# ChuRuaNh0/Image_Restoration

Hardware: AMD Instinct MI355X
Metric: images/sec (128x128->512x512 x4 SR, 23-block RRDBNet) (higher is better)
Workload: dtype f32

## Files before the change

### image_restoration_amd/csrc/conv_wino_f32.hip

```cpp
#include <stdlib.h>

#include <type_traits>

#include "sr_internal.h"

typedef float f32x4 __attribute__((ext_vector_type(4)));
typedef float f32x16 __attribute__((ext_vector_type(16)));

namespace {

struct WinoParams {
  const float* in;
  const float* u;
  const float* bias;
  float* out;
  const float* res1;
  const float* res2;
  long long in_ns, out_ns, res1_ns, res2_ns;
  int cin_blocks, cout_blocks;
  int in_h, in_w;
  int H, W;
  int tiles_x, tiles_y;
  int src_shift;
  int res_cb1;
  float slope, alpha, beta1, beta2;
#ifdef SR_WINO_STAMP
  unsigned long long* stamps;
#endif
};

#ifdef SR_WINO_STAMP
#define WINO_STAMP(k)                                                                                               \
  do {                                                                                                              \
    if (p.stamps && wave == 0 && lane == 0)                                                                         \
      p.stamps[(size_t)(blockIdx.y * gridDim.x + blockIdx.x) * 8 + (k)] = __builtin_amdgcn_s_memtime();             \
  } while (0)
#else
#define WINO_STAMP(k) \
  do {                \
  } while (0)
#endif

constexpr int XROW = 66;

template <int NW>
constexpr int wino_x_bytes() {
  return (((2 * NW + 2) * XROW * 32 + NW * 1024 - 1) / (NW * 1024)) * (NW * 1024);
}
template <int NW>
constexpr int wino_lds_bytes() {
  return 3 * wino_x_bytes<NW>() + 2 * 16 * 1024;
}

template <int NW, int HF>
__device__ __forceinline__ void conv_wino_tile_f32(const WinoParams p, char* smem, const int wave) {
  constexpr int NV = 2 * NW;
  constexpr int XPIX = (2 * NW + 2) * XROW;
  constexpr int XBYTES = wino_x_bytes<NW>();
  constexpr int NXU = (XPIX * 32 + 1023) / 1024, NWU = 16;
  constexpr int NXR = (NXU + NV - 1) / NV, NWR = NWU / NV;
  static_assert(NV * 8192 <= 3 * XBYTES, "the exchange of the output transform lives in the X buffers");

  int t;
  {
    const int nwg = gridDim.x, b = blockIdx.x;
    const int xcd = b & 7, q = nwg >> 3, r = nwg & 7;
    t = (xcd < r ? xcd * (q + 1) : r * (q + 1) + (xcd - r) * q) + (b >> 3);
  }
  const int tx = t % p.tiles_x;
  t /= p.tiles_x;
  const int ty = t % p.tiles_y;
  const int n = t / p.tiles_y;
  const int cog = blockIdx.y;

  const int lane = threadIdx.x & 63;
  WINO_STAMP(0);
  const int prow = wave - HF * NW;
  const int j = lane & 31, h = lane >> 5;
  const int x0 = tx * 64, y0 = ty * (2 * NW);
  const int HWin = p.in_h * p.in_w;
  const float* in_n = p.in + (long long)n * p.in_ns;
  const float* ug = p.u + (size_t)cog * p.cin_blocks * (NWU * 256);

  unsigned xvo[NXR];
#pragma unroll
  for (int r = 0; r < NXR; ++r) {
    const int u = r * NV + wave;
    const int q = u * 64 + lane;
    const int pix = q >> 1, half = q & 1;
    const int row = pix / XROW, col = pix - row * XROW;
    const int gy = y0 - 1 + row, gx = x0 - 1 + col;
    const bool valid = pix < XPIX && gy >= 0 && gy < p.H && gx >= 0 && gx < p.W;
    const int sy = gy >> p.src_shift, sx = gx >> p.src_shift;
    const int hsw = half ^ ((col >> 3) & 1);
    xvo[r] = valid ? (unsigned)((sy * p.in_w + sx) * 8 + hsw * 4) * 4u : 0xfffffff0u;
  }
  const __amdgpu_buffer_rsrc_t x_rs =
      __builtin_amdgcn_make_buffer_rsrc((void*)in_n, 0, (unsigned)((long long)p.cin_blocks * HWin * 32), 0x00020000);
  const __amdgpu_buffer_rsrc_t u_rs =
      __builtin_amdgcn_make_buffer_rsrc((void*)ug, 0, (unsigned)((long long)p.cin_blocks * NWU * 1024), 0x00020000);
  const unsigned uvo = (lane ^ ((lane >> 4) & 1)) * 16;
  auto stage_x = [&](int buf, int cb) {
    char* xs = smem + buf * XBYTES;
    const unsigned xso = (unsigned)cb * (unsigned)HWin * 32u;
#pragma unroll
    for (int r = 0; r < NXR; ++r) {
      const int u = r * NV + wave;
      if ((r + 1) * NV <= NXU || u < NXU)
        __builtin_amdgcn_raw_ptr_buffer_load_lds(x_rs, (__attribute__((address_space(3))) void*)(xs + u * 1024), 16, xvo[r], xso, 0, 0);
    }
  };
  auto stage_u = [&](int buf, int cb) {
    char* us = smem + 3 * XBYTES + buf * (NWU * 1024);
    const unsigned uso = (unsigned)cb * (NWU * 1024u);
#pragma unroll
    for (int r = 0; r < NWR; ++r) {
      const int u = r * NV + wave;
      __builtin_amdgcn_raw_ptr_buffer_load_lds(u_rs, (__attribute__((address_space(3))) void*)(us + u * 1024), 16, uvo, uso + u * 1024u, 0, 0);
    }
  };

  f32x16 acc[8];
#pragma unroll
  for (int a = 0; a < 8; ++a)
#pragma unroll
    for (int e = 0; e < 16; ++e) acc[a][e] = 0.f;

  int xlane[4];
#pragma unroll
  for (int c = 0; c < 4; ++c) xlane[c] = ((2 * prow + HF) * XROW + 2 * j + c) * 32 + ((h ^ (((2 * j + c) >> 3) & 1)) * 16);
  const int ulane = HF * 8 * 1024 + j * 32 + ((h ^ ((j >> 3) & 1)) * 16);

  f32x4 tr[2][4], v[8];
  auto rows = [&](int buf) {
    const char* xb = smem + buf * XBYTES;
#pragma unroll
    for (int c = 0; c < 4; ++c) {
      const f32x4 e0 = *(const f32x4*)(xb + xlane[c]);
      const f32x4 e1 = *(const f32x4*)(xb + xlane[c] + XROW * 32);
      const f32x4 e2 = *(const f32x4*)(xb + xlane[c] + 2 * XROW * 32);
      if constexpr (HF == 0) {
        tr[0][c] = e0 - e2;
        tr[1][c] = e1 + e2;
      } else {
        tr[0][c] = e1 - e0;
        tr[1][c] = e0 - e2;
      }
    }
  };
  auto cols = [&](int r) {
    v[r * 4 + 0] = tr[r][0] - tr[r][2];
    v[r * 4 + 1] = tr[r][1] + tr[r][2];
    v[r * 4 + 2] = tr[r][2] - tr[r][1];
    v[r * 4 + 3] = tr[r][1] - tr[r][3];
  };

  const int nchunk = p.cin_blocks;
  stage_x(0, 0);
  stage_u(0, 0);
  if (nchunk > 1) stage_x(1, 1);
  __syncthreads();
  WINO_STAMP(1);
  rows(0);
#pragma unroll
  for (int r = 0; r < 2; ++r) cols(r);
  int xb2 = 2 % 3, xb1 = 1;
  auto chunk = [&](int c, auto more_t, auto more2_t) {
    constexpr bool more = decltype(more_t)::value, more2 = decltype(more2_t)::value;
    const char* us = smem + 3 * XBYTES + (c & 1) * (NWU * 1024) + ulane;
    f32x4 a[2][4];
#pragma unroll
    for (int q = 0; q < 4; ++q) a[0][q] = *(const f32x4*)(us + q * 1024);
#pragma unroll
    for (int g = 0; g < 2; ++g) {
      if (g == 0) {
#pragma unroll
        for (int q = 0; q < 4; ++q) a[1][q] = *(const f32x4*)(us + (4 + q) * 1024);
        if constexpr (more2) stage_x(xb2, c + 2);
        if constexpr (more) stage_u((c + 1) & 1, c + 1);
      }
#pragma unroll
      for (int s = 0; s < 4; ++s)
#pragma unroll
        for (int q = 0; q < 4; ++q)
          acc[g * 4 + q] = __builtin_amdgcn_mfma_f32_32x32x2f32(a[g][q][s], v[g * 4 + q][s], acc[g * 4 + q], 0, 0, 0);
      if constexpr (more) {
        if (g == 0) rows(xb1);
        else cols(0);
      }
      __builtin_amdgcn_sched_barrier(0);
    }
    if constexpr (more) cols(1);
    __syncthreads();
    xb1 = xb2;
    xb2 = xb2 == 2 ? 0 : xb2 + 1;
  };
  using yes = std::true_type;
  using no = std::false_type;
  for (int c = 0; c + 2 < nchunk; ++c) chunk(c, yes{}, yes{});
  if (nchunk > 1) chunk(nchunk - 2, yes{}, no{});
  chunk(nchunk - 1, no{}, no{});
  WINO_STAMP(2);

  f32x16 ra[2][2];
#pragma unroll
  for (int r = 0; r < 2; ++r) {
    ra[r][0] = (acc[r * 4 + 0] + acc[r * 4 + 1]) + acc[r * 4 + 2];
    ra[r][1] = (acc[r * 4 + 1] - acc[r * 4 + 2]) - acc[r * 4 + 3];
  }

  f32x16 yv[2];
  {
    char* mine = smem + wave * 8192 + lane * 16;
    const char* theirs = smem + (HF ? wave - NW : wave + NW) * 8192 + lane * 16;
#pragma unroll
    for (int c = 0; c < 2; ++c)
#pragma unroll
      for (int k = 0; k < 4; ++k) {
        f32x4 o;
#pragma unroll
        for (int e = 0; e < 4; ++e) o[e] = ra[1 - HF][c][k * 4 + e];
        *(f32x4*)(mine + (c * 4 + k) * 1024) = o;
      }
    __syncthreads();
#pragma unroll
    for (int c = 0; c < 2; ++c) {
      f32x16 rb;
#pragma unroll
      for (int k = 0; k < 4; ++k) {
        const f32x4 o = *(const f32x4*)(theirs + (c * 4 + k) * 1024);
#pragma unroll
        for (int e = 0; e < 4; ++e) rb[k * 4 + e] = o[e];
      }
      if constexpr (HF == 0) yv[c] = (ra[0][c] + ra[1][c]) + rb;
      else yv[c] = (rb - ra[0][c]) - ra[1][c];
    }
  }

  WINO_STAMP(3);

  const long long HW = (long long)p.H * p.W;
  const int y = y0 + 2 * prow + HF;
#pragma unroll
  for (int dx = 0; dx < 2; ++dx) {
    const int x = x0 + 2 * j + dx;
    if (y >= p.H || x >= p.W) continue;
    const long long pixoff = (long long)y * p.W + x;
#pragma unroll
    for (int g = 0; g < 4; ++g) {
      const int cb = cog * 4 + g;
      if (cb >= p.cout_blocks) continue;
      f32x4 o;
#pragma unroll
      for (int e = 0; e < 4; ++e) o[e] = yv[dx][g * 4 + e];
      const long long off = (cb * HW + pixoff) * 8 + h * 4;
      if (p.bias) o += *(const f32x4*)(p.bias + cb * 8 + h * 4);
#pragma unroll
      for (int e = 0; e < 4; ++e) o[e] = o[e] > 0.f ? o[e] : o[e] * p.slope;
      o *= p.alpha;
      if (p.res1 && cb < p.res_cb1) o += p.beta1 * *(const f32x4*)(p.res1 + (long long)n * p.res1_ns + off);
      if (p.res2 && cb < p.res_cb1) o += p.beta2 * *(const f32x4*)(p.res2 + (long long)n * p.res2_ns + off);
      *(f32x4*)(p.out + (long long)n * p.out_ns + off) = o;
    }
  }
  WINO_STAMP(4);
}

template <int NW>
__global__ __launch_bounds__(NW * 128, 2) void conv_wino_f32_kernel(const WinoParams p) {
  extern __shared__ __attribute__((aligned(16))) char smem[];
  const int wave = __builtin_amdgcn_readfirstlane(threadIdx.x >> 6);
  if (wave < NW) conv_wino_tile_f32<NW, 0>(p, smem, wave);
  else conv_wino_tile_f32<NW, 1>(p, smem, wave);
}

#ifdef SR_WINO_STAMP
unsigned long long* g_wino_stamps = nullptr;
#endif

template <int NW>
int launch_wino(const WinoParams& p0, const sr_conv3x3_desc* d, hipStream_t stream) {
  WinoParams p = p0;
#ifdef SR_WINO_STAMP
  p.stamps = g_wino_stamps;
#endif
  p.tiles_x = sr::cdiv(p.W, 64);
  p.tiles_y = sr::cdiv(p.H, 2 * NW);
  constexpr int lds = wino_lds_bytes<NW>();
  auto kern = conv_wino_f32_kernel<NW>;
  if (int rc = sr::ensure_dynamic_lds((const void*)kern, lds)) return rc;
  const int groups = d->cout / 32;
  const bool prof = sr::prof_on();
  if (prof) {
    sr_launch_record r = {};
    r.kernel_id = NW == 4 ? 106 : NW == 2 ? 107 : 108;
    r.cin = d->cin_real > 0 ? d->cin_real : d->cin_pad;
    r.cout = d->cout;
    r.n = d->n;
    r.h = p.H;
    r.w = p.W;
    const double px = (double)d->n * p.H * p.W;
    const double patches = (double)d->n * ((p.H + 1) / 2) * ((p.W + 1) / 2);
    r.flops = 2.0 * 16 * d->cin_pad * d->cout * patches;
    double fl = (double)d->n * p.in_h * p.in_w * r.cin + px * r.cout;
    if (d->res1) fl += px * r.cout;
    if (d->res2) fl += px * r.cout;
    r.bytes = 4.0 * fl;
    sr::prof_begin(stream, r);
  }
  hipLaunchKernelGGL(kern, dim3(p.tiles_x * p.tiles_y * d->n, groups), dim3(NW * 128), lds, stream, p);
  if (prof) sr::prof_end(stream);
  SR_CHECK_LAUNCH("conv_wino_f32 launch");
  return SR_OK;
}

int g_wino_mode = -1;

}

namespace sr {

int wino_f32_mode() {
  if (g_wino_mode < 0) {
    const char* e = getenv("SR_F32_WINOGRAD");
    g_wino_mode = (e && *e) ? atoi(e) : 1;
    if (g_wino_mode < 0 || g_wino_mode > 4) g_wino_mode = 1;
  }
  return g_wino_mode;
}

bool wino_f32_weights_eligible(int cout, int cin) { return cin >= 8 && cout > 0 && cout % 32 == 0; }

size_t wino_f32_image_floats(int cout, int cin_pad) { return (size_t)cout * cin_pad * 16; }

int conv3x3_wino_f32(const sr_conv3x3_desc* d, const float* image, hipStream_t stream, bool any_size) {
  SR_CHECK_ARG(d != nullptr && image != nullptr, "conv3x3_wino_f32: null argument");
  SR_CHECK_ARG(d->in && d->out, "conv3x3_wino_f32: null in/out");
  SR_CHECK_ARG(d->cin_pad > 0 && d->cin_pad % 8 == 0, "conv3x3_wino_f32: cin_pad=%d must be a positive multiple of 8", d->cin_pad);
  SR_CHECK_ARG(d->cout > 0 && d->n > 0 && d->in_h > 0 && d->in_w > 0, "conv3x3_wino_f32: bad shape");
  SR_CHECK_ARG(((uintptr_t)d->in | (uintptr_t)image | (uintptr_t)d->out | (uintptr_t)d->res1 | (uintptr_t)d->res2 | (uintptr_t)d->bpacked) % 16 == 0,
               "conv3x3_wino_f32: pointers must be 16-byte aligned");
  const int cin = d->cin_real > 0 ? d->cin_real : d->cin_pad;
  if (!wino_f32_weights_eligible(d->cout, cin) || d->out_nchw || d->accumulate || d->mask_src || d->s2_channels || d->out_unshuffle2 ||
      d->res1_u2 || d->res1_keep_sign || (d->upsample != 0 && d->upsample != 1))
    return SR_WINO_NOT_ELIGIBLE;
  WinoParams p = {};
  p.in = d->in;
  p.u = image;
  p.bias = d->bpacked;
  p.out = d->out;
  p.res1 = d->res1;
  p.res2 = d->res2;
  p.in_ns = d->in_img_stride;
  p.out_ns = d->out_img_stride;
  p.res1_ns = d->res1_img_stride;
  p.res2_ns = d->res2_img_stride;
  p.cin_blocks = d->cin_pad / 8;
  p.cout_blocks = d->cout / 8;
  p.in_h = d->in_h;
  p.in_w = d->in_w;
  p.src_shift = d->upsample ? 1 : 0;
  p.H = d->in_h << p.src_shift;
  p.W = d->in_w << p.src_shift;
  p.res_cb1 = d->res_cbn > 0 ? d->res_cbn : (1 << 30);
  p.slope = d->act_slope;
  p.alpha = d->alpha;
  p.beta1 = d->beta1;
  p.beta2 = d->beta2;
  const long long blocks = p.cout_blocks > p.cin_blocks ? p.cout_blocks : p.cin_blocks;
  if ((long long)p.H * p.W * 32 * blocks >= (1ll << 31) || (long long)p.in_h * p.in_w * 32 * blocks >= (1ll << 31))
    return SR_WINO_NOT_ELIGIBLE;
  const int mode = wino_f32_mode();
  if (!any_size && mode < 2 && (long long)p.H * p.W < 128 * 128) return SR_WINO_NOT_ELIGIBLE;
  const long long rows2 = cdiv(p.H, 4), rows1 = cdiv(p.H, 2);
  const long long per_row = (long long)cdiv(p.W, 64) * d->n * (d->cout / 32) * launch_concurrency();
  if (per_row * rows1 >= (1ll << 31)) return SR_WINO_NOT_ELIGIBLE;
  const int nw = mode >= 2 ? (mode == 2 ? 4 : mode == 3 ? 2 : 1) : rows2 * per_row >= 256 ? 2 : 1;
  return nw == 4 ? launch_wino<4>(p, d, stream) : nw == 2 ? launch_wino<2>(p, d, stream) : launch_wino<1>(p, d, stream);
}

}

extern "C" int sr_dev_set_wino_f32(int mode) {
  g_wino_mode = (mode >= 0 && mode <= 4) ? mode : 1;
  return SR_OK;
}

#ifdef SR_WINO_STAMP
extern "C" int sr_dev_set_wino_stamps(unsigned long long* buf) {
  g_wino_stamps = buf;
  return SR_OK;
}
#endif

extern "C" int sr_dev_conv3x3_wino_f32(const sr_conv3x3_desc* d, const float* wino_image, void* stream) {
  return sr::conv3x3_wino_f32(d, wino_image, (hipStream_t)stream, true);
}

extern "C" size_t sr_dev_conv3x3_wino_packed_floats(int cout, int cin_pad) {
  return (cout > 0 && cin_pad > 0 && cout % 32 == 0 && cin_pad % 8 == 0) ? sr::wino_f32_image_floats(cout, cin_pad) : 0;
}

extern "C" int sr_dev_conv3x3_wino_pack_f32(const float* weight, int cout, int cin, int first_seg, int seg, float* wino_image,
                                            void* stream) {
  SR_CHECK_ARG(weight && wino_image && sr::wino_f32_weights_eligible(cout, cin), "sr_dev_conv3x3_wino_pack_f32: bad argument");
  const int cin_pad = sr_conv3x3_cin_pad(cin, first_seg, seg);
  SR_CHECK_ARG(cin_pad > 0, "sr_dev_conv3x3_wino_pack_f32: cin=%d is not first_seg=%d + k*seg=%d", cin, first_seg, seg);
  std::vector<sr::PackEntry> tab(1);
  sr::PackEntry& e = tab[0];
  e = sr::PackEntry{};
  e.kind = 3;
  e.w[0] = weight;
  e.out = wino_image;
  e.cout = cout;
  e.cin = cin;
  e.first_seg = first_seg;
  e.seg = seg > 0 ? seg : 1;
  e.cin_pad = cin_pad;
  return sr::pack_table_run(tab, wino_image, sr::wino_f32_image_floats(cout, e.cin_pad) * sizeof(float), false, (hipStream_t)stream);
}

extern "C" size_t sr_dev_conv3x3_wino_pack_bytes(int cout, int cin_pad) {
  const size_t f = sr_dev_conv3x3_wino_packed_floats(cout, cin_pad);
  return f ? f * sizeof(float) + sr::pack_table_bytes(1) : 0;
}
```

Baseline: 411.8.

## Add nearest-upsample Winograd variant skipping zero tiles and stage residual via LDS

Adds a specialised Winograd F(2x2,3x3) kernel for the nearest-neighbour x2 upsample conv (src_shift==1). It exploits duplicated input rows and columns so that 7 of the 16 transformed elements are zero, and skips their loads, transforms, MFMAs and the cross-half exchange. For NW<=2 it also prefetches the res1 residual tile into the X region of LDS during the last chunk, and moves the output-transform exchange into the U buffers. The cost is more template instantiations and LDS reuse constraints, and the UP2 algebra must be correct.

```diff
diff --git a/image_restoration_amd/csrc/conv_wino_f32.hip b/image_restoration_amd/csrc/conv_wino_f32.hip
--- a/image_restoration_amd/csrc/conv_wino_f32.hip
+++ b/image_restoration_amd/csrc/conv_wino_f32.hip
@@ -52,14 +52,19 @@
   return 3 * wino_x_bytes<NW>() + 2 * 16 * 1024;
 }
 
-template <int NW, int HF>
+template <int NW, int HF, bool UP2>
 __device__ __forceinline__ void conv_wino_tile_f32(const WinoParams p, char* smem, const int wave) {
   constexpr int NV = 2 * NW;
   constexpr int XPIX = (2 * NW + 2) * XROW;
   constexpr int XBYTES = wino_x_bytes<NW>();
   constexpr int NXU = (XPIX * 32 + 1023) / 1024, NWU = 16;
   constexpr int NXR = (NXU + NV - 1) / NV, NWR = NWU / NV;
-  static_assert(NV * 8192 <= 3 * XBYTES, "the exchange of the output transform lives in the X buffers");
+  constexpr bool RES_LDS = NW <= 2;
+  constexpr int RBYTES = NV * 8 * 1024;
+  constexpr int XCH = RES_LDS ? 3 * XBYTES : 0;
+  auto used = [](int a) constexpr { return !UP2 || ((a & 3) != 2 && !(HF == 1 && (a >> 2) == 0)); };
+  static_assert(RES_LDS ? (NV * 8192 <= 2 * NWU * 1024 && RBYTES <= 3 * XBYTES) : NV * 8192 <= 3 * XBYTES,
+                "the exchange of the output transform lives in the U buffers (NW <= 2: the res1 tile takes the X region) or the X region");
 
   int t;
   {
@@ -120,6 +125,26 @@
     }
   };
 
+  const int res_cbn = p.res_cb1 < p.cout_blocks ? p.res_cb1 : p.cout_blocks;
+  auto stage_res = [&]() {
+    const long long HWo = (long long)p.H * p.W;
+    const __amdgpu_buffer_rsrc_t r_rs = __builtin_amdgcn_make_buffer_rsrc((void*)(p.res1 + (long long)n * p.res1_ns), 0,
+                                                                          (unsigned)(res_cbn * HWo * 32), 0x00020000);
+    const int gy = y0 + wave;
+#pragma unroll
+    for (int dx = 0; dx < 2; ++dx) {
+      const int gx = x0 + 2 * (lane & 31) + dx;
+      const unsigned rvo = (gy < p.H && gx < p.W) ? ((unsigned)gy * (unsigned)p.W + (unsigned)gx) * 32u + (unsigned)(lane >> 5) * 16u : 0xfffffff0u;
+#pragma unroll
+      for (int g = 0; g < 4; ++g) {
+        const int cb = cog * 4 + g, u = (wave * 4 + g) * 2 + dx;
+        if (cb < res_cbn)
+          __builtin_amdgcn_raw_ptr_buffer_load_lds(r_rs, (__attribute__((address_space(3))) void*)(smem + u * 1024), 16, rvo,
+                                                   (unsigned)cb * (unsigned)HWo * 32u, 0, 0);
+      }
+    }
+  };
+
   f32x16 acc[8];
 #pragma unroll
   for (int a = 0; a < 8; ++a)
@@ -136,23 +161,43 @@
     const char* xb = smem + buf * XBYTES;
 #pragma unroll
     for (int c = 0; c < 4; ++c) {
-      const f32x4 e0 = *(const f32x4*)(xb + xlane[c]);
-      const f32x4 e1 = *(const f32x4*)(xb + xlane[c] + XROW * 32);
-      const f32x4 e2 = *(const f32x4*)(xb + xlane[c] + 2 * XROW * 32);
-      if constexpr (HF == 0) {
-        tr[0][c] = e0 - e2;
-        tr[1][c] = e1 + e2;
+      if constexpr (UP2) {
+        if (c == 2) continue;
+        const f32x4 e0 = *(const f32x4*)(xb + xlane[c]);
+        if constexpr (HF == 0) {
+          const f32x4 e1 = *(const f32x4*)(xb + xlane[c] + XROW * 32);
+          tr[0][c] = e0 - e1;
+          tr[1][c] = e1 + e1;
+        } else {
+          const f32x4 e2 = *(const f32x4*)(xb + xlane[c] + 2 * XROW * 32);
+          tr[1][c] = e0 - e2;
+        }
       } else {
-        tr[0][c] = e1 - e0;
-        tr[1][c] = e0 - e2;
+        const f32x4 e0 = *(const f32x4*)(xb + xlane[c]);
+        const f32x4 e1 = *(const f32x4*)(xb + xlane[c] + XROW * 32);
+        const f32x4 e2 = *(const f32x4*)(xb + xlane[c] + 2 * XROW * 32);
+        if constexpr (HF == 0) {
+          tr[0][c] = e0 - e2;
+          tr[1][c] = e1 + e2;
+        } else {
+          tr[0][c] = e1 - e0;
+          tr[1][c] = e0 - e2;
+        }
       }
     }
   };
   auto cols = [&](int r) {
-    v[r * 4 + 0] = tr[r][0] - tr[r][2];
-    v[r * 4 + 1] = tr[r][1] + tr[r][2];
-    v[r * 4 + 2] = tr[r][2] - tr[r][1];
-    v[r * 4 + 3] = tr[r][1] - tr[r][3];
+    if constexpr (UP2) {
+      if (HF == 1 && r == 0) return;
+      v[r * 4 + 0] = tr[r][0] - tr[r][1];
+      v[r * 4 + 1] = tr[r][1] + tr[r][1];
+      v[r * 4 + 3] = tr[r][1] - tr[r][3];
+    } else {
+      v[r * 4 + 0] = tr[r][0] - tr[r][2];
+      v[r * 4 + 1] = tr[r][1] + tr[r][2];
+      v[r * 4 + 2] = tr[r][2] - tr[r][1];
+      v[r * 4 + 3] = tr[r][1] - tr[r][3];
+    }
   };
 
   const int nchunk = p.cin_blocks;
@@ -170,12 +215,14 @@
     const char* us = smem + 3 * XBYTES + (c & 1) * (NWU * 1024) + ulane;
     f32x4 a[2][4];
 #pragma unroll
-    for (int q = 0; q < 4; ++q) a[0][q] = *(const f32x4*)(us + q * 1024);
+    for (int q = 0; q < 4; ++q)
+      if (used(q)) a[0][q] = *(const f32x4*)(us + q * 1024);
 #pragma unroll
     for (int g = 0; g < 2; ++g) {
       if (g == 0) {
 #pragma unroll
-        for (int q = 0; q < 4; ++q) a[1][q] = *(const f32x4*)(us + (4 + q) * 1024);
+        for (int q = 0; q < 4; ++q)
+          if (used(4 + q)) a[1][q] = *(const f32x4*)(us + (4 + q) * 1024);
         if constexpr (more2) stage_x(xb2, c + 2);
         if constexpr (more) stage_u((c + 1) & 1, c + 1);
       }
@@ -183,7 +230,8 @@
       for (int s = 0; s < 4; ++s)
 #pragma unroll
         for (int q = 0; q < 4; ++q)
-          acc[g * 4 + q] = __builtin_amdgcn_mfma_f32_32x32x2f32(a[g][q][s], v[g * 4 + q][s], acc[g * 4 + q], 0, 0, 0);
+          if (used(g * 4 + q))
+            acc[g * 4 + q] = __builtin_amdgcn_mfma_f32_32x32x2f32(a[g][q][s], v[g * 4 + q][s], acc[g * 4 + q], 0, 0, 0);
       if constexpr (more) {
         if (g == 0) rows(xb1);
         else cols(0);
@@ -199,6 +247,11 @@
   using no = std::false_type;
   for (int c = 0; c + 2 < nchunk; ++c) chunk(c, yes{}, yes{});
   if (nchunk > 1) chunk(nchunk - 2, yes{}, no{});
+  {
+    const bool res_lds = RES_LDS && p.res1;
+    if (nchunk == 1 && res_lds) __syncthreads();
+    if (res_lds) stage_res();
+  }
   chunk(nchunk - 1, no{}, no{});
   WINO_STAMP(2);
 
@@ -211,24 +264,28 @@
 
   f32x16 yv[2];
   {
-    char* mine = smem + wave * 8192 + lane * 16;
-    const char* theirs = smem + (HF ? wave - NW : wave + NW) * 8192 + lane * 16;
-#pragma unroll
-    for (int c = 0; c < 2; ++c)
-#pragma unroll
-      for (int k = 0; k < 4; ++k) {
-        f32x4 o;
-#pragma unroll
-        for (int e = 0; e < 4; ++e) o[e] = ra[1 - HF][c][k * 4 + e];
-        *(f32x4*)(mine + (c * 4 + k) * 1024) = o;
-      }
+    char* mine = smem + XCH + wave * 8192 + lane * 16;
+    const char* theirs = smem + XCH + (HF ? wave - NW : wave + NW) * 8192 + lane * 16;
+    constexpr bool ROW2_ZERO = UP2;
+    if constexpr (!(ROW2_ZERO && HF == 1)) {
+#pragma unroll
+      for (int c = 0; c < 2; ++c)
+#pragma unroll
+        for (int k = 0; k < 4; ++k) {
+          f32x4 o;
+#pragma unroll
+          for (int e = 0; e < 4; ++e) o[e] = ra[1 - HF][c][k * 4 + e];
+          *(f32x4*)(mine + (c * 4 + k) * 1024) = o;
+        }
+    }
     __syncthreads();
 #pragma unroll
     for (int c = 0; c < 2; ++c) {
       f32x16 rb;
 #pragma unroll
       for (int k = 0; k < 4; ++k) {
-        const f32x4 o = *(const f32x4*)(theirs + (c * 4 + k) * 1024);
+        f32x4 o = {0.f, 0.f, 0.f, 0.f};
+        if constexpr (!(ROW2_ZERO && HF == 0)) o = *(const f32x4*)(theirs + (c * 4 + k) * 1024);
 #pragma unroll
         for (int e = 0; e < 4; ++e) rb[k * 4 + e] = o[e];
       }
@@ -258,7 +315,10 @@
 #pragma unroll
       for (int e = 0; e < 4; ++e) o[e] = o[e] > 0.f ? o[e] : o[e] * p.slope;
       o *= p.alpha;
-      if (p.res1 && cb < p.res_cb1) o += p.beta1 * *(const f32x4*)(p.res1 + (long long)n * p.res1_ns + off);
+      if (p.res1 && cb < p.res_cb1) {
+        if constexpr (RES_LDS) o += p.beta1 * *(const f32x4*)(smem + (((2 * prow + HF) * 4 + g) * 2 + dx) * 1024 + lane * 16);
+        else o += p.beta1 * *(const f32x4*)(p.res1 + (long long)n * p.res1_ns + off);
+      }
       if (p.res2 && cb < p.res_cb1) o += p.beta2 * *(const f32x4*)(p.res2 + (long long)n * p.res2_ns + off);
       *(f32x4*)(p.out + (long long)n * p.out_ns + off) = o;
     }
@@ -270,8 +330,16 @@
 __global__ __launch_bounds__(NW * 128, 2) void conv_wino_f32_kernel(const WinoParams p) {
   extern __shared__ __attribute__((aligned(16))) char smem[];
   const int wave = __builtin_amdgcn_readfirstlane(threadIdx.x >> 6);
-  if (wave < NW) conv_wino_tile_f32<NW, 0>(p, smem, wave);
-  else conv_wino_tile_f32<NW, 1>(p, smem, wave);
+  if (wave < NW) conv_wino_tile_f32<NW, 0, false>(p, smem, wave);
+  else conv_wino_tile_f32<NW, 1, false>(p, smem, wave);
+}
+
+template <int NW>
+__global__ __launch_bounds__(NW * 128, 2) void conv_wino_up2_f32_kernel(const WinoParams p) {
+  extern __shared__ __attribute__((aligned(16))) char smem[];
+  const int wave = __builtin_amdgcn_readfirstlane(threadIdx.x >> 6);
+  if (wave < NW) conv_wino_tile_f32<NW, 0, true>(p, smem, wave);
+  else conv_wino_tile_f32<NW, 1, true>(p, smem, wave);
 }
 
 #ifdef SR_WINO_STAMP
@@ -287,7 +355,8 @@
   p.tiles_x = sr::cdiv(p.W, 64);
   p.tiles_y = sr::cdiv(p.H, 2 * NW);
   constexpr int lds = wino_lds_bytes<NW>();
-  auto kern = conv_wino_f32_kernel<NW>;
+  const bool up2 = p.src_shift == 1;
+  auto kern = up2 ? conv_wino_up2_f32_kernel<NW> : conv_wino_f32_kernel<NW>;
   if (int rc = sr::ensure_dynamic_lds((const void*)kern, lds)) return rc;
   const int groups = d->cout / 32;
   const bool prof = sr::prof_on();
@@ -301,7 +370,7 @@
     r.w = p.W;
     const double px = (double)d->n * p.H * p.W;
     const double patches = (double)d->n * ((p.H + 1) / 2) * ((p.W + 1) / 2);
-    r.flops = 2.0 * 16 * d->cin_pad * d->cout * patches;
+    r.flops = 2.0 * (up2 ? 9 : 16) * d->cin_pad * d->cout * patches;
     double fl = (double)d->n * p.in_h * p.in_w * r.cin + px * r.cout;
     if (d->res1) fl += px * r.cout;
     if (d->res2) fl += px * r.cout;
```

Measured after the change: 418.5, median of 6. 1.6% higher.
